# heimrih/polar_code

Measured on AMD Instinct MI355X. Metric: decoded frames/sec, P(128,64)+CRC24 SCL L=8 @ Eb/N0=5 dB; FER match, higher is better.
Workload: dtype f64

## Files before the change

### polar_code_amd/csrc/scl128_lane.hip

```cpp
#ifndef PSCL_LANE_REMAP
#define PSCL_LANE_REMAP 0
#endif
#if PSCL_LANE_REMAP
#define PSCL_LANE_FRAME_MIRROR 0x140
#endif
#include "scl_lane.h"

#ifdef PSCL_LANE_F32_UNIT
using lane_llr_t = float;
#define scl_lane_kernel scl_lane_kernel_f32
#else
using lane_llr_t = double;
#endif

namespace {

#ifndef PSCL_LANE_REG56
#define PSCL_LANE_REG56 1
#endif

#ifndef PSCL_LANE_FRES8
#define PSCL_LANE_FRES8 8
#endif
#ifndef PSCL_LANE_FRES4
#define PSCL_LANE_FRES4 24
#endif

template <int LMAX>
struct LaneLayout {
    static constexpr int G = LMAX;
    static constexpr int F = 64 / G;
    static constexpr int LOG_G = __builtin_ctz(G);
    static constexpr int OFF3 = 0;
    static constexpr int OFF4 = OFF3 + 16 * LMAX;
    static constexpr int OFF5 = OFF4 + 8 * LMAX;
    static constexpr int OFF6 = OFF5 + 4 * LMAX;
    static constexpr int OFFX = PSCL_LANE_REG56 ? OFF4 : OFF6;
    static constexpr int RAW = PSCL_LANE_REG56 ? OFF5 : OFF6 + 2 * LMAX;
    static constexpr int FRES = LMAX == 8 ? PSCL_LANE_FRES8 : PSCL_LANE_FRES4;
    static constexpr int FSTRIDE = RAW + (((FRES - RAW) % 32) + 32) % 32;
    static constexpr int FSTRIDE_FS = FSTRIDE >= 128 ? FSTRIDE : FSTRIDE + 32;
    static constexpr int FSTRIDE_EX = FSTRIDE + 8;
};

__device__ __forceinline__ uint64_t flip_order_key(double q) {
    if (q == 0.0) q = 0.0;
    const uint64_t u = pscl_asu64(q);
    return (u >> 63) ? ~u : (u | 0x8000000000000000ULL);
}

#ifndef PSCL_LANE_CREG4
#define PSCL_LANE_CREG4 1
#endif

#ifndef PSCL_LANE_ABL
#define PSCL_LANE_ABL 0
#endif

#ifndef PSCL_LANE_WAVES_PER_EU
#define PSCL_LANE_WAVES_PER_EU 2
#endif

#ifndef PSCL_LANE_U0T
#define PSCL_LANE_U0T 1
#endif
#ifndef PSCL_LANE_GSPLIT
#define PSCL_LANE_GSPLIT 1
#endif

__device__ __forceinline__ void tx_frame_words(const pscl_decode_params& P, uint64_t fr, uint64_t (&m)[2],
                                               uint64_t (&raw)[2], uint64_t (&x)[2]) {
    const u32x4 rb = philox4x32(u32x4{(uint32_t)fr, (uint32_t)(fr >> 32), 0xffffffffu, 0u}, P.tx_k0, P.tx_k1);
    raw[0] = ((uint64_t)rb.y << 32) | rb.x;
    raw[1] = ((uint64_t)rb.w << 32) | rb.z;
    const int kp = P.tx_kp, nbp = (kp + 7) >> 3, nb = (P.K + 7) >> 3;
    m[0] = kp >= 64 ? raw[0] : (raw[0] & ((1ULL << kp) - 1));
    m[1] = kp > 64 ? (raw[1] & ((kp >= 128) ? ~0ULL : ((1ULL << (kp - 64)) - 1))) : 0;
    uint32_t rem = 0;
    for (int k = 0; k < nbp; ++k) rem ^= P.tx_crctab[k * 256 + (uint32_t)((m[k >> 3] >> (8 * (k & 7))) & 255u)];
    if (P.tx_crc_deg) {
        const uint64_t rw = (uint64_t)rem;
        if (kp < 64) {
            m[0] |= rw << kp;
            if (kp + P.tx_crc_deg > 64) m[1] |= rw >> (64 - kp);
        } else {
            m[1] |= rw << (kp - 64);
        }
    }
    x[0] = x[1] = 0;
    for (int k = 0; k < nb; ++k) {
        const uint32_t v = (uint32_t)((m[k >> 3] >> (8 * (k & 7))) & 255u);
        x[0] ^= P.tx_xtab[(k * 256 + v) * 2];
        x[1] ^= P.tx_xtab[(k * 256 + v) * 2 + 1];
    }
}

#ifndef PSCL_FS_WAVES
#define PSCL_FS_WAVES 3
#endif
#ifndef PSCL_TX_WAVES
#define PSCL_TX_WAVES 3
#endif
template <int LMAX, int CODE, bool FS = false, bool TXF = false, bool FP = false, bool EX = false, bool RL = false>
__global__ void __launch_bounds__(64, TXF ? (LMAX == 8 ? PSCL_TX_WAVES : 2)
                                           : (FS && !FP && !EX && LMAX == 8) ? PSCL_FS_WAVES : PSCL_LANE_WAVES_PER_EU)
scl_lane_kernel(const pscl_decode_params P) {
    static_assert(LMAX == 4 || LMAX == 8, "the lane-per-path decoder is built for L = 4 and 8");
    static_assert(!TXF || (!FS && CODE == 1), "fused TX: plain decodes of the (128,64) code");
    static_assert(!FP || (FS && CODE == 1), "fused post pass: the FS instance of the (128,64) code");
    static_assert(!EX || (!TXF && !FP), "the exact instance: plain re-decodes and forced-bit retry decodes");
    static_assert(!RL || (!FS && !TXF && !FP && !EX), "the row-list form: plain screening decodes");
    using Ly = LaneLayout<LMAX>;
    constexpr int G = Ly::G, F = Ly::F, LOG_G = Ly::LOG_G;
    constexpr int EPL = 16 / G;
    constexpr uint32_t GM = (1u << G) - 1u;
    constexpr int K = kSpecK[CODE], PW = (K + 63) / 64;
    constexpr uint64_t info0 = kSpecInfo[CODE][0], info1 = kSpecInfo[CODE][1];
    extern __shared__ __attribute__((aligned(16))) unsigned char smem[];
    double* const A = reinterpret_cast<double*>(smem);
    const int lane = threadIdx.x & 63;
    constexpr bool REMAP = PSCL_LANE_REMAP && G == 8 && !EX;
    const int rq = (lane >> 2) & 3, inner = (rq == 1 || rq == 2) ? 1 : 0;
    const int fl = REMAP ? 2 * (lane >> 4) + inner : lane >> LOG_G;
    const int p = REMAP ? (lane & 3) + 4 * (rq & 1) : lane & (G - 1);
    const int lane_lo = REMAP ? (lane & ~15) + (inner ? 8 : 0) : lane & ~(G - 1);
    const int lane_hi = REMAP ? (lane & ~15) + (inner ? 4 : 12) : lane_lo + 4;
    auto lane_of = [&](uint32_t q) -> int { return REMAP ? (q < 4u ? lane_lo + (int)q : lane_hi + (int)q - 4) : lane_lo + (int)q; };
    double* const Af = A + fl * (FP ? Ly::FSTRIDE_FS : EX ? Ly::FSTRIDE_EX : Ly::FSTRIDE);
    int* const sl = reinterpret_cast<int*>(Af + Ly::FSTRIDE);
    const uint8_t* const GT = reinterpret_cast<const uint8_t*>(P.epi_table);
    const uint32_t* const ST = reinterpret_cast<const uint32_t*>(GT + 16 * 256);
    auto hiw = [](double m) { return (uint32_t)(pscl_asu64(m) >> 32); };
    constexpr bool BITS = !FS && !EX && PSCL_LANE_BITS;
    constexpr bool PLAIN = !FS && !EX && !TXF;
    constexpr bool U0T = PLAIN && PSCL_LANE_U0T;
    constexpr bool GSPLIT = PLAIN && PSCL_LANE_GSPLIT && (LMAX == 8 || PSCL_LANE_CREG4);
    constexpr double MARGIN = BITS ? PSCL_TAIL2_MARGIN : PSCL_TAIL_ABS_MARGIN;
    auto hiw_up = [&](double m) {
        double r;
        asm("v_fma_f64 %0, %1, %2, %3" : "=v"(r) : "v"(m), "s"(1.0 + 0x1p-40), "v"(MARGIN));
        return hiw(r);
    };
    auto frame_bits = [&](uint64_t m) -> uint32_t {
        if constexpr (REMAP) return ((uint32_t)(m >> lane_lo) & 15u) | (((uint32_t)(m >> lane_hi) & 15u) << 4);
        return (uint32_t)(m >> lane_lo) & GM;
    };

    int cfe = 0, cbe = 0, cpe = 0, cpb = 0;
    int tufe = 0, tube = 0;
    int pdecodes = 0;
    int bpre[PSCL_DL_NSEG + 1];
    int64_t Bn = P.B;
    if constexpr (FS) {
        const int64_t tot = pscl_bucket_prefix(P.bcount, P.bcap, bpre);
        Bn = tot < P.B ? tot : P.B;
    } else if constexpr (EX) {
        if (P.d_count) Bn = *P.d_count < P.B ? (int64_t)*P.d_count : P.B;
    } else if constexpr (RL) {
        Bn = *P.d_count < P.B ? (int64_t)*P.d_count : P.B;
    }
    for (int64_t f0 = (int64_t)blockIdx.x * F; f0 < Bn; f0 += (int64_t)gridDim.x * F) {
        const int64_t fi = f0 + fl;
        const bool fvalid = fi < Bn;
        const int64_t fsafe = fvalid ? fi : f0;
        int64_t f = fi, frow = fsafe;
        int seg0 = 0;
        if constexpr (FS) {
            f = pscl_elist_entry(P, fsafe, bpre);
            seg0 = pscl_bucket_of(f0, bpre);
            frow = P.fidx[f];
        } else if constexpr (EX) {
            if (P.fidx) frow = P.fidx[fsafe];
        } else if constexpr (RL) {
            frow = P.fidx[fsafe];
        }
        constexpr bool RM = CODE == 2;
        const lane_llr_t* chan = reinterpret_cast<const lane_llr_t*>(P.llr) + frow * (RM ? (int64_t)P.rm_E : (int64_t)kN);
        auto chan_at = [&](int i) -> double { return RM ? nr_stage(chan, P.rm_src[i], P.rm_E, kN) : (double)chan[i]; };
        constexpr bool CREG = G == 8 || PSCL_LANE_CREG4 || TXF;
        double c[8 * EPL];
        uint64_t tm[2] = {0, 0}, traw[2] = {0, 0}, tx[2] = {0, 0};
        const uint64_t tfr = TXF ? (uint64_t)(P.tx_frame0 + fsafe) : 0ULL;
        if constexpr (TXF) tx_frame_words(P, tfr, tm, traw, tx);
        auto gen_chan = [&](double* v, uint64_t fr) {
#pragma unroll
            for (int k = 0; k < EPL; ++k)
#pragma unroll
                for (int j = 0; j < 4; ++j) {
                    const uint32_t blk = (uint32_t)(p + G * k + 16 * j);
                    const u32x4 rn = philox4x32(u32x4{(uint32_t)fr, (uint32_t)(fr >> 32), blk, 0u}, P.tx_k0, P.tx_k1);
                    double z[2];
                    bm_pair(((uint64_t)rn.y << 32) | rn.x, ((uint64_t)rn.w << 32) | rn.z, z[0], z[1]);
#pragma unroll
                    for (int h = 0; h < 2; ++h) {
                        const double sym = ((tx[h] >> blk) & 1ULL) ? -1.0 : 1.0;
                        v[8 * k + j + 4 * h] = (sym + P.tx_sigma * z[h]) * P.tx_scale;
                    }
                    __builtin_amdgcn_sched_barrier(0);
                }
        };
        auto load_chan = [&]() {
            if constexpr (TXF) {
                gen_chan(c, tfr);
                if constexpr (BITS)
#pragma unroll
                    for (int m = 0; m < 8 * EPL; ++m) c[m] = c[m] * PSCL_LOG2E_F64;
            } else {
#pragma unroll
                for (int k = 0; k < EPL; ++k)
#pragma unroll
                    for (int m = 0; m < 8; ++m) c[8 * k + m] = BITS ? chan_at(p + G * k + 16 * m) * PSCL_LOG2E_F64
                                                                    : chan_at(p + G * k + 16 * m);
            }
        };
        load_chan();
        uint32_t ah[4 * EPL];
#pragma unroll
        for (int m = 0; m < 4 * EPL; ++m) {
            ah[m] = GSPLIT ? hiw(c[8 * (m >> 2) + (m & 3)]) : 0u;
            if constexpr (GSPLIT) asm volatile("" : "+v"(ah[m]));
        }
        if constexpr (TXF) {
            if (P.tx_upart) {
                uint32_t berr = 0;
                for (int cb = p; 2 * cb < P.tx_kp; cb += G) {
                    const u32x4 rn = philox4x32(u32x4{(uint32_t)tfr, (uint32_t)(tfr >> 32), 0x40000000u + (uint32_t)cb, 0u},
                                                P.tx_k0, P.tx_k1);
                    double z[2];
                    bm_pair(((uint64_t)rn.y << 32) | rn.x, ((uint64_t)rn.w << 32) | rn.z, z[0], z[1]);
#pragma unroll
                    for (int h = 0; h < 2; ++h) {
                        const int q = 2 * cb + h;
                        if (q < P.tx_kp) {
                            const uint32_t bit = (uint32_t)((traw[q >> 6] >> (q & 63)) & 1ULL);
                            const double y = (bit ? -1.0 : 1.0) + P.tx_unc_sigma * z[h];
                            berr += ((y < 0.0) ? 1u : 0u) != bit ? 1u : 0u;
                        }
                    }
                }
                berr = frame_sum<G>(berr);
                if (fvalid && p == 0) {
                    tufe += berr ? 1 : 0;
                    tube += (int)berr;
                }
            }
        }
        double cs = fabs(c[0]);
#pragma unroll
        for (int m = 1; m < 8 * EPL; ++m) cs = cs + fabs(c[m]);
        uint64_t amb = EX ? 0ULL : wmask(!(cs < (BITS ? PSCL_TAIL2_CHAN_SUM : 0x1p25)));
        const uint64_t vmask = wmask(fvalid);

        double metric = 0.0;
        uint64_t u0 = 0, u1 = 0;
        uint32_t tab = 0;
        uint32_t lastbit = 0;
        double r5[4] = {0.0, 0.0, 0.0, 0.0}, r6[2] = {0.0, 0.0};
        uint64_t fm0 = 0, fm1 = 0, fv0 = 0, fv1 = 0;
        int lcnt = 0;
        if constexpr (FS) {
            const uint64_t* fr = P.force + f * 2 * PW;
            fm0 = fr[0];
            fv0 = fr[PW];
            if (PW > 1) {
                fm1 = fr[1];
                fv1 = fr[PW + 1];
            }
            if (seg0 > 0) {
                metric = P.warm_metric[f * PSCL_DL_NSEG + seg0];
                const int lo = 16 * seg0;
                u0 = P.warm_u[2 * f];
                u1 = P.warm_u[2 * f + 1];
                if (lo < 64) {
                    u0 &= (1ULL << lo) - 1ULL;
                    u1 = 0;
                } else {
                    u1 = lo == 64 ? 0ULL : (u1 & ((1ULL << (lo - 64)) - 1ULL));
                }
            }
        }

        auto phase = [&](auto PC) {
            constexpr int phi = decltype(PC)::value;
            constexpr int t = phi & 15;
            constexpr int start = t ? kn - __builtin_ctz((unsigned)t) : ((phi >> 4) ? 3 - __builtin_ctz((unsigned)(phi >> 4)) : 1);
            constexpr bool is_info = ((phi < 64 ? info0 : info1) >> (phi & 63)) & 1;
            constexpr int jb = phi < 64 ? __builtin_popcountll(info0 & ((1ULL << (phi & 63)) - 1))
                                        : __builtin_popcountll(info0) + __builtin_popcountll(info1 & ((1ULL << (phi & 63)) - 1));
            constexpr int cnt = jb >= LOG_G ? LMAX : (1 << jb);
#ifdef PSCL_PHASE_MARKERS
            asm volatile("; PHASE %0" ::"n"(t));
#endif

            if constexpr (start <= 3 && !(PSCL_LANE_ABL & 4)) {
                constexpr bool r1 = phi >= 64, r2 = (phi >> 5) & 1, r3 = (phi >> 4) & 1;
                if constexpr (!CREG && phi > 0) load_chan();
                uint4* const xs = reinterpret_cast<uint4*>(Af + Ly::OFFX);
                if constexpr (r1 || r2 || r3) {
                    uint64_t X1 = 0;
                    uint32_t X2 = 0, X3 = 0;
                    if constexpr (U0T && phi == 64) u0 = polar_transform64(u0);
                    if (r1) X1 = U0T ? u0 : polar_transform64(u0);
                    if (r2) {
                        constexpr int lo = phi - (phi & 31) - 32;
                        X2 = polar_transform32((uint32_t)((lo >= 64 ? u1 : u0) >> (lo & 63)));
                    }
                    if (r3) {
                        constexpr int lo = phi - 16;
                        X3 = polar_transform16((uint32_t)((lo >= 64 ? u1 : u0) >> (lo & 63)) & 0xffffu);
                    }
                    xs[p] = make_uint4((uint32_t)X1, (uint32_t)(X1 >> 32), X2, (X2 >> 16) | (X3 << 16));
                    wave_lds_fence();
                }
                constexpr bool shared2 = !r1 && !r2;
                double d1l[EPL][4], d2s[EPL][2];
#pragma unroll
                for (int h = 0; h < EPL; ++h) {
#pragma unroll
                    for (int m = 0; m < 4; ++m) d1l[h][m] = r1 ? 0.0 : f_minsum(c[8 * h + m], c[8 * h + m + 4]);
#pragma unroll
                    for (int s2 = 0; s2 < 2; ++s2) d2s[h][s2] = shared2 ? f_minsum(d1l[h][s2], d1l[h][s2 + 2]) : 0.0;
                }
                constexpr int npaths = FS ? LMAX : cnt;
#pragma unroll
                for (int q0 = 0; q0 < npaths; ++q0) {
                    const int q = npaths == LMAX ? ((q0 + p) & (LMAX - 1)) : q0;
                    uint64_t x1 = 0, x23 = 0;
                    if constexpr (r1 || r2 || r3) {
                        const uint4 xv = xs[q];
                        x1 = ((uint64_t)xv.y << 32) | xv.x;
                        x23 = ((uint64_t)xv.w << 32) | xv.z;
                    }
                    double d3[EPL];
#pragma unroll
                    for (int h = 0; h < EPL; ++h) {
                        const uint32_t e = (uint32_t)(p + G * h);
                        const uint64_t s1[2] = {r1 ? x1 << (31u - e) : 0ULL, r1 ? x1 << (15u - e) : 0ULL};
                        const uint64_t s2w = r2 ? x23 << (31u - e) : 0ULL;
                        double d1[4];
#pragma unroll
                        for (int m = 0; m < 4; ++m)
                            d1[m] = !r1 ? d1l[h][m]
                                    : GSPLIT ? g_node_bit31_split(c[8 * h + m], ah[4 * h + m], c[8 * h + m + 4],
                                                                  (uint32_t)(s1[m & 1] >> (32 * (m >> 1))))
                                             : g_node_bit31(c[8 * h + m], c[8 * h + m + 4], (uint32_t)(s1[m & 1] >> (32 * (m >> 1))));
                        double d2[2];
#pragma unroll
                        for (int s2 = 0; s2 < 2; ++s2)
                            d2[s2] = shared2 ? d2s[h][s2]
                                             : (r2 ? g_node_bit31(d1[s2], d1[s2 + 2], (uint32_t)(s2w >> (32 * s2))) : f_minsum(d1[s2], d1[s2 + 2]));
                        d3[h] = r3 ? g_node_wbit(d2[0], d2[1], (uint32_t)(x23 >> 32), e + 16) : f_minsum(d2[0], d2[1]);
                    }
#pragma unroll
                    for (int h = 0; h < EPL / 2; ++h)
                        *reinterpret_cast<double2*>(Af + Ly::OFF3 + ((p + G * h) * LMAX + q) * 2) = make_double2(d3[h], d3[h + EPL / 2]);
                }
                wave_lds_fence();
            }
            if constexpr (start <= 6) {
                uint32_t xsb = 0;
                if constexpr (phi && start >= 4) {
                    constexpr int w = 1 << (kn - start), lo = phi - w;
                    static_assert(phi <= 64 || lo >= 64, "u0 is not read bit-wise after phase 64 (PSCL_LANE_U0T)");
                    xsb = polar_transform8((uint32_t)((lo >= 64 ? u1 : u0) >> (lo & 63)) & ((1u << w) - 1u));
                }
                static_for<3>([&](auto DI) {
                    constexpr int D = 4 + decltype(DI)::value;
                    if constexpr (D >= start) {
                        constexpr int W = 1 << (kn - D), HW = W / 2;
                        constexpr int OFF_IN = D == 4 ? Ly::OFF3 : (D == 5 ? Ly::OFF4 : Ly::OFF5);
                        constexpr int OFF_OUT = D == 4 ? Ly::OFF4 : (D == 5 ? Ly::OFF5 : Ly::OFF6);
                        constexpr bool first = D == start || (D == 4 && start < 4);
                        constexpr bool is_g = D == start && phi != 0;
                        if constexpr (PSCL_LANE_REG56 && D == 6) {
#pragma unroll
                            for (int k = 0; k < 2; ++k)
                                r6[k] = is_g ? g_node(r5[k], r5[k + 2], (xsb >> k) & 1u) : f_minsum(r5[k], r5[k + 2]);
                        } else {
                            const int sin = first ? slot_at(tab, D - 1) : p;
                            const int sin_eff = (D == 4 && start <= 3) ? p : sin;
                            const double* in = Af + OFF_IN + sin_eff * 2;
                            double o[W];
#pragma unroll
                            for (int k = 0; k < W; ++k) {
                                const double2 ab = *reinterpret_cast<const double2*>(in + k * LMAX * 2);
                                o[k] = is_g ? g_node(ab.x, ab.y, (xsb >> k) & 1u) : f_minsum(ab.x, ab.y);
                            }
                            if constexpr (PSCL_LANE_REG56 && D == 5) {
#pragma unroll
                                for (int k = 0; k < 4; ++k) r5[k] = o[k];
                            } else {
                                double* out = Af + OFF_OUT + p * 2;
                                if constexpr (HW >= 1) {
#pragma unroll
                                    for (int k = 0; k < (HW ? HW : 1); ++k)
                                        *reinterpret_cast<double2*>(out + k * LMAX * 2) = make_double2(o[k], o[k + HW]);
                                }
                                wave_lds_fence();
                            }
                        }
                    }
                });
                constexpr int s0 = start < 3 ? 3 : start;
                constexpr uint32_t mask = (0xffffu << (4 * (s0 - 3))) & 0xffffu;
                tab = (tab & ~mask) | ((uint32_t)p * 0x1111u & mask);
            }
            const double2 lab = PSCL_LANE_REG56 ? make_double2(r6[0], r6[1])
                                                : *reinterpret_cast<const double2*>(Af + Ly::OFF6 + (start <= 6 ? p : slot_at(tab, 6)) * 2);
            constexpr bool C6 = PSCL_LANE_REG56 && (t % 2 == 0), C5 = PSCL_LANE_REG56 && (t % 4 <= 1);
            auto carry = [&](int src, double (&q5)[4], double (&q6)[2]) {
                if constexpr (C5)
#pragma unroll
                    for (int k = 0; k < 4; ++k) q5[k] = shfl_f64(r5[k], src);
                if constexpr (C6)
#pragma unroll
                    for (int k = 0; k < 2; ++k) q6[k] = shfl_f64(r6[k], src);
            };
            auto take = [&](const double (&q5)[4], const double (&q6)[2]) {
                if constexpr (C5)
#pragma unroll
                    for (int k = 0; k < 4; ++k) r5[k] = q5[k];
                if constexpr (C6)
#pragma unroll
                    for (int k = 0; k < 2; ++k) r6[k] = q6[k];
            };
            const double lam = (phi & 1) ? g_node(lab.x, lab.y, lastbit) : f_minsum(lab.x, lab.y);
            const double Lt = EX ? pscl_softplus_tail_bf(lam, P.exp_table) : BITS ? pscl_softplus_tail2(lam) : pscl_softplus_tail_abs(lam);
            if constexpr (EX) {
                const int ncur = FS ? (1 << lcnt) : cnt;
                const bool live = p < ncur;
                const bool zl = lam == 0.0;
                auto pull_path = [&](int src) {
                    u0 = shfl_u64(u0, src);
                    if constexpr (phi >= 64) u1 = shfl_u64(u1, src);
                    tab = bperm32(tab, src);
                    double q5[4], q6[2];
                    carry(src, q5, q6);
                    take(q5, q6);
                };
                if constexpr (!is_info) {
                    metric = zl ? metric + PSCL_LOGE2 : metric + (relu_neg(lam) + Lt);
                    lastbit = 0;
                    const double pm = shfl_f64(metric, p > 0 ? lane - 1 : lane);
                    if ((wmask(live && pm > metric) & vmask) == 0) return;
                    const double mk = live ? metric : __builtin_inf();
                    uint32_t r = 0;
#pragma unroll
                    for (int sx = 1; sx < G; ++sx) {
                        const double om = shfl_f64(mk, lane ^ sx);
                        r += (om < mk || (om == mk && (p ^ sx) < p)) ? 1u : 0u;
                    }
                    if (live) sl[r] = p;
                    wave_lds_fence();
                    const int src = lane_lo + sl[p & (ncur - 1)];
                    wave_lds_fence();
                    metric = shfl_f64(metric, src);
                    pull_path(src);
                    return;
                }
                const bool neg = lam < 0.0;
                const double mgd = metric + Lt, mbd = metric + (fabs(lam) + Lt);
                double m0 = neg ? mbd : mgd, m1 = neg ? mgd : mbd;
                if (zl) {
                    m0 = metric + PSCL_LOGE2;
                    m1 = m0;
                }
                bool forced = false;
                uint32_t fbit = 0;
                if constexpr (FS) {
                    const uint64_t fmw = jb < 64 ? fm0 : fm1, fvw = jb < 64 ? fv0 : fv1;
                    forced = ((fmw >> (jb & 63)) & 1ULL) != 0;
                    fbit = (uint32_t)((fvw >> (jb & 63)) & 1ULL);
                }
                const double top = shfl_f64(mgd, lane_lo + LMAX - 1), pg = shfl_f64(mgd, p > 0 ? lane - 1 : lane);
                const bool badk = zl || (p > 0 && pg > mgd) || !(mbd > top);
                const bool fast = forced ? ncur == 1 : (ncur == LMAX && frame_bits(wmask(badk)) == 0);
                uint32_t b = forced ? fbit : sign_bit(lam);
                if ((wmask(!fast) & vmask) != 0) {
                    const bool v0 = live && (!forced || fbit == 0u), v1 = live && (!forced || fbit == 1u);
                    const int ncnt = forced ? ncur : (2 * ncur < LMAX ? 2 * ncur : LMAX);
                    const double k0 = v0 ? m0 : __builtin_inf(), k1 = v1 ? m1 : __builtin_inf();
                    uint32_t r0 = k1 < k0 ? 1u : 0u, r1 = k0 <= k1 ? 1u : 0u;
#pragma unroll
                    for (int sx = 1; sx < G; ++sx) {
                        const double o0 = shfl_f64(k0, lane ^ sx), o1 = shfl_f64(k1, lane ^ sx);
                        const bool lt = (p ^ sx) < p;
                        r0 += ((o0 < k0 || (o0 == k0 && lt)) ? 1u : 0u) + ((o1 < k0 || (o1 == k0 && lt)) ? 1u : 0u);
                        r1 += ((o0 < k1 || (o0 == k1 && lt)) ? 1u : 0u) + ((o1 < k1 || (o1 == k1 && lt)) ? 1u : 0u);
                    }
                    if (!fast) {
                        if (v0 && r0 < (uint32_t)ncnt) sl[r0] = 2 * p;
                        if (v1 && r1 < (uint32_t)ncnt) sl[r1] = 2 * p + 1;
                    }
                    wave_lds_fence();
                    const int code = fast ? 2 * p + (int)b : sl[p & (ncnt - 1)];
                    wave_lds_fence();
                    const int src = lane_lo + (code >> 1);
                    b = (uint32_t)code & 1u;
                    const double p0 = shfl_f64(m0, src), p1 = shfl_f64(m1, src);
                    metric = b ? p1 : p0;
                    pull_path(src);
                    if constexpr (FS) lcnt += (!fast && !forced && ncur < LMAX) ? 1 : 0;
                } else {
                    metric = b ? m1 : m0;
                }
                if (phi < 64) u0 |= (uint64_t)b << phi; else u1 |= (uint64_t)b << (phi - 64);
                lastbit = b;
                return;
            }
            if constexpr (!is_info) {
                metric = metric + (relu_neg(lam) + Lt);
                lastbit = 0;
                return;
            }
            const double mg = metric + Lt, mb = mg + fabs(lam);
            const uint32_t gbit = sign_bit(lam);
            if constexpr (FS) {
                const uint64_t fmw = jb < 64 ? fm0 : fm1, fvw = jb < 64 ? fv0 : fv1;
                const bool forced = ((fmw >> (jb & 63)) & 1ULL) != 0;
                const uint32_t fbit = (uint32_t)((fvw >> (jb & 63)) & 1ULL);
                const bool full = !forced && lcnt == LOG_G, grow = !forced && lcnt < LOG_G;
                const int cntf = 1 << lcnt;
                const double m1 = gbit ? mg : mb;
                double nm = forced ? (fbit == gbit ? mg : mb) : (grow ? (gbit ? mb : mg) : mg);
                uint32_t b = forced ? fbit : (grow ? 0u : gbit);
                bool pull = grow && (p & cntf) != 0;
                int src = grow ? lane_of((uint32_t)(p & (cntf - 1))) : lane;
                const uint64_t fullm = wmask(full) & vmask;
                const uint32_t kgu = hiw_up(mg), kb = hiw(mb);
                const uint32_t mx = frame_max<G>(kgu);
                const bool bad = kb <= mx;
                const uint64_t badm = wmask(bad);
                if ((badm & fullm) != 0) {
                    const uint32_t bad8 = frame_bits(badm);
                    if ((wmask(__builtin_popcount(bad8) > 1) & fullm) == 0) {
                        const uint32_t kg = hiw(mg);
                        const uint32_t gmaxh = frame_max<G>(kg);
                        const bool ismax = kg == gmaxh;
                        const uint32_t nmax = frame_sum<G>(ismax ? 1u : 0u);
                        const uint32_t g2u = frame_max<G>(ismax ? 0u : kgu);
                        const uint32_t wu = frame_max<G>(bad ? hiw_up(mb) : 0u);
                        const bool swap = bad8 != 0;
                        amb |= wmask(full && swap && !(nmax == 1u && g2u < gmaxh && wu < gmaxh)) & vmask;
                        if (full && swap && ismax) {
                            pull = true;
                            src = lane_of(__builtin_ctz(bad8 | (1u << G)) & (G - 1));
                        }
                    } else {
                        const uint32_t kg = hiw(mg);
                        bool keep_g, win_b;
                        select_survivors<G, LMAX>(kg, kb, keep_g, win_b);
                        const uint32_t kbu = hiw_up(mb);
                        const uint32_t su = keep_g ? (win_b ? kbu : kgu) : (win_b ? kbu : 0u);
                        const uint32_t nmk = keep_g ? (win_b ? 0xffffffffu : kb) : kg;
                        const uint32_t nsurv = frame_sum<G>((keep_g ? 1u : 0u) + (win_b ? 1u : 0u));
                        const uint32_t smax = frame_max<G>(su), nmin = frame_min<G>(nmk);
                        amb |= wmask(full && !(nsurv == (uint32_t)LMAX && nmin > smax)) & vmask;
                        const uint32_t f8 = frame_bits(wmask(!keep_g)), w8 = frame_bits(wmask(win_b));
                        const uint32_t jj = __builtin_popcount(f8 & ((1u << p) - 1u));
                        const int rsrc = lane_of(nth_set_bit8(w8, jj));
                        if (full && !keep_g) {
                            pull = true;
                            src = rsrc;
                        }
                    }
                }
                if (wmask(pull) != 0) {
                    const uint64_t pubm = pscl_asu64(full ? mb : m1);
                    const uint32_t tw = tab | ((full ? (gbit ^ 1u) : 1u) << 31);
                    const uint64_t pm = shfl_u64(pubm, src);
                    const uint64_t pu0 = shfl_u64(u0, src);
                    const uint64_t pu1 = phi >= 64 ? shfl_u64(u1, src) : 0ULL;
                    const uint32_t ptw = bperm32(tw, src);
                    double q5[4], q6[2];
                    carry(src, q5, q6);
                    if (pull) {
                        nm = pscl_asf64(pm);
                        u0 = pu0;
                        u1 = pu1;
                        tab = ptw & 0x7fffffffu;
                        b = ptw >> 31;
                        take(q5, q6);
                    }
                }
                metric = nm;
                if (phi < 64) u0 |= (uint64_t)b << phi; else u1 |= (uint64_t)b << (phi - 64);
                lastbit = b;
                lcnt += grow ? 1 : 0;
                return;
            }
            if constexpr (cnt < LMAX) {
                const double m0 = gbit ? mb : mg, m1 = gbit ? mg : mb;
                const int src = lane_of((uint32_t)(p & (cnt - 1)));
                const uint32_t b = (p & cnt) ? 1u : 0u;
                const uint64_t pm1 = shfl_u64(pscl_asu64(m1), src);
                metric = b ? pscl_asf64(pm1) : m0;
                u0 = shfl_u64(u0, src);
                if (phi >= 64) u1 = shfl_u64(u1, src);
                tab = bperm32(tab, src);
                double q5[4], q6[2];
                carry(src, q5, q6);
                take(q5, q6);
                if (phi < 64) u0 |= (uint64_t)b << phi; else u1 |= (uint64_t)b << (phi - 64);
                lastbit = b;
                return;
            }
            const uint32_t kgu = hiw_up(mg), kb = hiw(mb);
            const uint32_t mx = frame_max<G>(kgu);
            const bool bad = kb <= mx;
            const uint64_t badm = wmask(bad);
#ifdef PSCL_STATS
            const bool one = (wmask(__builtin_popcount(frame_bits(badm)) > 1) & vmask) == 0;
            if (lane == 0 && P.counters) {
                atomicAdd(reinterpret_cast<unsigned long long*>(P.counters) + ((badm & vmask) == 0 ? 12 : (one ? 13 : 14)), 1ULL);
            }
#endif
            metric = mg;
            uint32_t b = gbit;
            if (!(PSCL_LANE_ABL & 2) && ((badm & vmask) != 0 || (PSCL_LANE_ABL & 1))) {
                const uint32_t bad8 = frame_bits(badm);
                bool pull;
                int src;
#if PSCL_LANE_SWAP
                if (!(PSCL_LANE_ABL & 1) && (wmask(__builtin_popcount(bad8) > 1) & vmask) == 0) {
                    const uint32_t kg = hiw(mg);
                    const uint32_t gmaxh = frame_max<G>(kg);
                    const bool ismax = kg == gmaxh;
                    const uint32_t nmax = __builtin_popcount(frame_bits(wmask(ismax)));
                    const bool g2ok = ismax || kgu < gmaxh;
                    const bool wok = !bad || hiw_up(mb) < gmaxh;
                    const bool swap = bad8 != 0;
                    amb |= wmask(swap && !(nmax == 1u && g2ok && wok)) & vmask;
                    src = lane_of(__builtin_ctz(bad8 | (1u << G)) & (G - 1));
                    pull = swap && ismax;
                } else
#endif
                {
                    const uint32_t kg = hiw(mg);
                    uint32_t rg, rbb;
                    rank_children<G>(kg, kb, rg, rbb);
                    const bool keep_g = rg < (uint32_t)LMAX;
                    const uint32_t f8 = frame_bits(wmask(!keep_g));
                    const uint32_t d = __builtin_popcount(f8);
                    const bool win_b = rbb < d;
                    const uint32_t w8 = frame_bits(wmask(win_b));
#if defined(PSCL_STATS) && PSCL_STATS == 2
                    {
                        const uint32_t dw = frame_sum<G>(win_b ? 1u : 0u);
                        const uint32_t nb = __builtin_popcount(bad8);
                        unsigned long long* C = reinterpret_cast<unsigned long long*>(P.counters);
                        if (p == 0 && fvalid && C) {
                            atomicAdd(C + 16 + (dw > 8u ? 8u : dw), 1ULL);
                            atomicAdd(C + 25 + nb, 1ULL);
                        }
                        uint32_t md = 0;
                        for (uint32_t k = 1; k <= 8; ++k)
                            if (wmask(dw >= k) & vmask) md = k;
                        if (lane == 0 && C) atomicAdd(C + 34 + md, 1ULL);
                    }
#endif
                    const uint32_t kbu = hiw_up(mb);
                    const uint32_t su = keep_g ? (win_b ? kbu : kgu) : (win_b ? kbu : 0u);
                    const uint32_t nm = keep_g ? (win_b ? 0xffffffffu : kb) : kg;
                    const uint32_t smax = frame_max<G>(su);
                    amb |= wmask(!((uint32_t)__builtin_popcount(w8) == d && nm > smax)) & vmask;
                    src = lane_of(matched_winner<G>(f8, w8, win_b, (uint32_t)p));
                    pull = !keep_g;
                }
                const int srce = pull ? src : lane;
                const uint64_t pmb = shfl_u64(pscl_asu64(mb), srce);
                const uint32_t ptw = bperm32(tab | ((gbit ^ 1u) << 31), srce);
                u0 = shfl_u64(u0, srce);
                if constexpr (phi >= 64) u1 = shfl_u64(u1, srce);
                tab = ptw & 0x7fffffffu;
                double q5[4], q6[2];
                carry(srce, q5, q6);
                take(q5, q6);
                if (pull) {
                    metric = pscl_asf64(pmb);
                    b = ptw >> 31;
                }
            }
            if (phi < 64) u0 |= (uint64_t)b << phi; else u1 |= (uint64_t)b << (phi - 64);
            lastbit = b;
        };
        if constexpr (FS) {
            auto seg = [&](auto SB) {
                static_for<16>([&](auto TC) { phase(std::integral_constant<int, decltype(SB)::value * 16 + decltype(TC)::value>{}); });
            };
            using std::integral_constant;
            switch (seg0) {
                case 0: seg(integral_constant<int, 0>{}); [[fallthrough]];
                case 1: seg(integral_constant<int, 1>{}); [[fallthrough]];
                case 2: seg(integral_constant<int, 2>{}); [[fallthrough]];
                case 3: seg(integral_constant<int, 3>{}); [[fallthrough]];
                case 4: seg(integral_constant<int, 4>{}); [[fallthrough]];
                case 5: seg(integral_constant<int, 5>{}); [[fallthrough]];
                case 6: seg(integral_constant<int, 6>{}); [[fallthrough]];
                default: seg(integral_constant<int, 7>{});
            }
        } else {
            static_for<kN>([&](auto PC) { phase(PC); });
        }

        auto fused_post = [&](bool x_amb, bool x_live, uint32_t x_keyb, uint32_t x_kbest, uint64_t x_ib0, uint64_t x_ib1,
                              uint64_t x_u0, uint64_t x_u1, int64_t x_frow, int64_t e, bool x_valid) {
            static_assert(!REMAP, "the fused post pass assumes frames of G consecutive lanes");
            const pscl_post_params& Q = P.fp;
            constexpr int NC = K / G;
            const uint32_t fl = (x_kbest < (uint32_t)LMAX ? PSCL_FLAG_CRC_PASS : 0u) | (x_kbest & (uint32_t)(LMAX - 1));
            const bool mine = x_valid && !x_amb;
            int nt = 0;
            uint64_t t0 = 0, t1 = 0;
            if (mine) {
                nt = Q.ntried[e];
                t0 = Q.tried[2 * e];
                t1 = Q.tried[2 * e + 1];
            }
            const uint32_t bfb = frame_bits(wmask(x_live && x_keyb == x_kbest));
            const int bsrc = lane_lo + (bfb ? __builtin_ctz(bfb) : 0);
            const uint64_t bi0 = shfl_u64(x_ib0, bsrc), bi1 = PW > 1 ? shfl_u64(x_ib1, bsrc) : 0ULL;
            const uint64_t bu0 = shfl_u64(x_u0, bsrc), bu1 = shfl_u64(x_u1, bsrc);
            if (mine && p == 0) {
                Q.best[x_frow * PW] = bi0;
                if (PW > 1) Q.best[x_frow * PW + 1] = bi1;
                Q.flags[x_frow] = (uint8_t)fl;
                if (Q.attempts) Q.attempts[x_frow] = nt + 1;
                ++pdecodes;
            }
            const bool more = mine && !(fl & PSCL_FLAG_CRC_PASS) && nt < Q.rounds;
            if (wmask(more) == 0) return;
            wave_lds_fence();
            {
                const double* crow = P.llr + x_frow * kN;
#pragma unroll
                for (int j = 0; j < kN / G; ++j) Af[p + G * j] = crow[p + G * j];
            }
            wave_lds_fence();
            auto stage = [](uint64_t x, int st) {
                const uint64_t M = st == 1 ? 0x5555555555555555ULL : st == 2 ? 0x3333333333333333ULL
                                 : st == 4 ? 0x0f0f0f0f0f0f0f0fULL : st == 8 ? 0x00ff00ff00ff00ffULL
                                 : st == 16 ? 0x0000ffff0000ffffULL : 0x00000000ffffffffULL;
                return x ^ ((x >> st) & M);
            };
            uint64_t X0 = bu0, X1 = bu1;
#pragma unroll
            for (int mm = 1; mm < kn; ++mm) {
                X0 = stage(X0, 1 << (mm - 1));
                X1 = stage(X1, 1 << (mm - 1));
            }
            static_for<kn>([&](auto DC) {
                constexpr int lw2 = kn - 1 - decltype(DC)::value, w2 = 1 << lw2;
                const bool act_l = w2 >= G || (p & w2) == 0;
                if (act_l) {
#pragma unroll 2
                    for (int j = 0; j < kN / G; ++j) {
                        const int q = p + G * j;
                        if (w2 >= G && (q & w2)) continue;
                        const double a = Af[q], b = Af[q + w2];
                        const uint32_t bit = (uint32_t)(((q >> 6) ? X1 : X0) >> (q & 63)) & 1u;
                        Af[q] = f_minsum(a, b);
                        Af[q + w2] = g_node(a, b, bit);
                    }
                }
                wave_lds_fence();
                if constexpr (lw2 > 0) {
                    X0 = stage(X0, w2 >> 1);
                    X1 = stage(X1, w2 >> 1);
                }
            });
            float qv[NC];
            double as = 0.0;
            uint64_t bk = ~0ULL;
            int bj = 0x7fffffff;
            auto seen_j = [&](int j) { return (((j < 64 ? t0 : t1) >> (j & 63)) & 1ULL) != 0; };
            auto argmin = [&]() {
                bk = ~0ULL;
                bj = 0x7fffffff;
#pragma unroll
                for (int i = 0; i < NC; ++i) {
                    const int j = p + G * i;
                    const uint64_t key = seen_j(j) ? ~0ULL : flip_order_key((double)qv[i]);
                    if (key < bk) {
                        bk = key;
                        bj = j;
                    }
                }
#pragma unroll
                for (int sft = 1; sft < G; sft <<= 1) {
                    const uint64_t ok = shfl_u64(bk, lane ^ sft);
                    const int oj = __shfl(bj, lane ^ sft);
                    if (ok < bk || (ok == bk && oj < bj)) {
                        bk = ok;
                        bj = oj;
                    }
                }
            };
            auto argmin_exact = [&]() {
                bk = ~0ULL;
                bj = 0x7fffffff;
#pragma unroll 1
                for (int i = 0; i < NC; ++i) {
                    const int j = p + G * i;
                    double qx = 0.0;
#pragma unroll 1
                    for (int k = 0; k < K; ++k) qx = qx + fabs(Af[Q.info_set[k]]) * Q.beta[k * K + j];
                    const uint64_t key = seen_j(j) ? ~0ULL : flip_order_key(qx);
                    if (key < bk) {
                        bk = key;
                        bj = j;
                    }
                }
#pragma unroll
                for (int sft = 1; sft < G; sft <<= 1) {
                    const uint64_t ok = shfl_u64(bk, lane ^ sft);
                    const int oj = __shfl(bj, lane ^ sft);
                    if (ok < bk || (ok == bk && oj < bj)) {
                        bk = ok;
// ... 380 lines not shown
```

### polar_code_amd/csrc/scl_lane.h

```cpp
#ifndef PSCL_SCL_LANE_H
#define PSCL_SCL_LANE_H

#include "scl128_impl.h"

#ifndef PSCL_LANE_SWAP
#define PSCL_LANE_SWAP 1
#endif


#ifndef PSCL_LANE_BITS
#define PSCL_LANE_BITS 1
#endif

namespace {

constexpr int kQX1 = 0xB1, kQX2 = 0x4E, kQX3 = 0x1B, kQID = 0xE4, kHMIR = 0x141;
#ifndef PSCL_LANE_FRAME_MIRROR
#define PSCL_LANE_FRAME_MIRROR 0x141
#endif
constexpr int kFMIR = PSCL_LANE_FRAME_MIRROR;

template <int CTRL>
__device__ __forceinline__ uint32_t dpp32(uint32_t v) {
    return (uint32_t)__builtin_amdgcn_mov_dpp((int)v, CTRL, 0xF, 0xF, true);
}

template <int CTRL>
__device__ __forceinline__ void rank_pair(uint32_t og, uint32_t ob, uint32_t kg, uint32_t kb, uint32_t& rg, uint32_t& rb) {
    uint32_t t;
    asm volatile(
        "s_nop 1\n\t"
        "v_sub_co_u32_dpp %0, vcc, %3, %5 quad_perm:[%7,%8,%9,%10] row_mask:0xf bank_mask:0xf\n\t"
        "v_addc_co_u32 %1, vcc, 0, %1, vcc\n\t"
        "v_sub_co_u32_dpp %0, vcc, %4, %5 quad_perm:[%7,%8,%9,%10] row_mask:0xf bank_mask:0xf\n\t"
        "v_addc_co_u32 %1, vcc, 0, %1, vcc\n\t"
        "v_sub_co_u32_dpp %0, vcc, %3, %6 quad_perm:[%7,%8,%9,%10] row_mask:0xf bank_mask:0xf\n\t"
        "v_addc_co_u32 %2, vcc, 0, %2, vcc\n\t"
        "v_sub_co_u32_dpp %0, vcc, %4, %6 quad_perm:[%7,%8,%9,%10] row_mask:0xf bank_mask:0xf\n\t"
        "v_addc_co_u32 %2, vcc, 0, %2, vcc"
        : "=&v"(t), "+v"(rg), "+v"(rb)
        : "v"(og), "v"(ob), "v"(kg), "v"(kb), "i"(CTRL & 3), "i"((CTRL >> 2) & 3), "i"((CTRL >> 4) & 3),
          "i"((CTRL >> 6) & 3)
        : "vcc");
}

template <int CTRL>
__device__ __forceinline__ void rank3(uint32_t og, uint32_t ob, uint32_t kg, uint32_t kb, uint32_t& rg, uint32_t& rbb) {
    uint32_t t;
    asm volatile(
        "s_nop 1\n\t"
        "v_sub_co_u32_dpp %0, vcc, %3, %5 quad_perm:[%7,%8,%9,%10] row_mask:0xf bank_mask:0xf\n\t"
        "v_addc_co_u32 %1, vcc, 0, %1, vcc\n\t"
        "v_sub_co_u32_dpp %0, vcc, %4, %5 quad_perm:[%7,%8,%9,%10] row_mask:0xf bank_mask:0xf\n\t"
        "v_addc_co_u32 %1, vcc, 0, %1, vcc\n\t"
        "v_sub_co_u32_dpp %0, vcc, %4, %6 quad_perm:[%7,%8,%9,%10] row_mask:0xf bank_mask:0xf\n\t"
        "v_addc_co_u32 %2, vcc, 0, %2, vcc"
        : "=&v"(t), "+v"(rg), "+v"(rbb)
        : "v"(og), "v"(ob), "v"(kg), "v"(kb), "i"(CTRL & 3), "i"((CTRL >> 2) & 3), "i"((CTRL >> 4) & 3),
          "i"((CTRL >> 6) & 3)
        : "vcc");
}

constexpr int kRMIR = 0x140;

__device__ __forceinline__ uint32_t xrow32(uint32_t v) { return (uint32_t)__shfl_xor((int)v, 16); }

template <int G>
__device__ __forceinline__ uint32_t frame_max(uint32_t v) {
    uint32_t o = dpp32<kQX1>(v);
    v = o > v ? o : v;
    o = dpp32<kQX2>(v);
    v = o > v ? o : v;
    if constexpr (G >= 8) {
        o = dpp32<G >= 16 ? kHMIR : kFMIR>(v);
        v = o > v ? o : v;
    }
    if constexpr (G >= 16) {
        o = dpp32<kRMIR>(v);
        v = o > v ? o : v;
    }
    if constexpr (G == 32) {
        o = xrow32(v);
        v = o > v ? o : v;
    }
    return v;
}
template <int G>
__device__ __forceinline__ uint32_t frame_min(uint32_t v) {
    uint32_t o = dpp32<kQX1>(v);
    v = o < v ? o : v;
    o = dpp32<kQX2>(v);
    v = o < v ? o : v;
    if constexpr (G >= 8) {
        o = dpp32<G >= 16 ? kHMIR : kFMIR>(v);
        v = o < v ? o : v;
    }
    if constexpr (G >= 16) {
        o = dpp32<kRMIR>(v);
        v = o < v ? o : v;
    }
    if constexpr (G == 32) {
        o = xrow32(v);
        v = o < v ? o : v;
    }
    return v;
}
template <int G>
__device__ __forceinline__ uint32_t frame_sum(uint32_t v) {
    v += dpp32<kQX1>(v);
    v += dpp32<kQX2>(v);
    if constexpr (G >= 8) v += dpp32<G >= 16 ? kHMIR : kFMIR>(v);
    if constexpr (G >= 16) v += dpp32<kRMIR>(v);
    if constexpr (G == 32) v += xrow32(v);
    return v;
}
template <int G>
__device__ __forceinline__ uint32_t frame_or(uint32_t v) {
    v |= dpp32<kQX1>(v);
    v |= dpp32<kQX2>(v);
    if constexpr (G >= 8) v |= dpp32<G >= 16 ? kHMIR : kFMIR>(v);
    if constexpr (G >= 16) v |= dpp32<kRMIR>(v);
    if constexpr (G == 32) v |= xrow32(v);
    return v;
}

#ifndef PSCL_LANE_RANK3
#define PSCL_LANE_RANK3 1
#endif
template <int G, int LMAX>
__device__ __forceinline__ void select_survivors(uint32_t kg, uint32_t kb, bool& keep_g, bool& win_b) {
#if PSCL_LANE_RANK3
    uint32_t rg = 0, rbb = 0;
    rank3<kQX1>(kg, kb, kg, kb, rg, rbb);
    rank3<kQX2>(kg, kb, kg, kb, rg, rbb);
    rank3<kQX3>(kg, kb, kg, kb, rg, rbb);
    if constexpr (G >= 8) {
        const uint32_t mkg = dpp32<G >= 16 ? kHMIR : kFMIR>(kg), mkb = dpp32<G >= 16 ? kHMIR : kFMIR>(kb);
        rank3<kQID>(mkg, mkb, kg, kb, rg, rbb);
        rank3<kQX1>(mkg, mkb, kg, kb, rg, rbb);
        rank3<kQX2>(mkg, mkb, kg, kb, rg, rbb);
        rank3<kQX3>(mkg, mkb, kg, kb, rg, rbb);
    }
    auto quads16 = [&](uint32_t ok, uint32_t ob) {
        rank3<kQID>(ok, ob, kg, kb, rg, rbb);
        rank3<kQX1>(ok, ob, kg, kb, rg, rbb);
        rank3<kQX2>(ok, ob, kg, kb, rg, rbb);
        rank3<kQX3>(ok, ob, kg, kb, rg, rbb);
    };
    if constexpr (G >= 16) {
        quads16(dpp32<kRMIR>(kg), dpp32<kRMIR>(kb));
        quads16(dpp32<kRMIR>(dpp32<kHMIR>(kg)), dpp32<kRMIR>(dpp32<kHMIR>(kb)));
    }
    if constexpr (G == 32) {
        const uint32_t xg = xrow32(kg), xb = xrow32(kb);
        quads16(xg, xb);
        quads16(dpp32<kHMIR>(xg), dpp32<kHMIR>(xb));
        quads16(dpp32<kRMIR>(xg), dpp32<kRMIR>(xb));
        quads16(dpp32<kRMIR>(dpp32<kHMIR>(xg)), dpp32<kRMIR>(dpp32<kHMIR>(xb)));
    }
    keep_g = rg < (uint32_t)LMAX;
    const uint32_t d = frame_sum<G>(keep_g ? 0u : 1u);
    win_b = rbb < d;
#else
    static_assert(G <= 8, "the two-rank selection is built for frames of at most 8 lanes");
    uint32_t rg = 0, rb = kg < kb ? 1u : 0u;
    rank_pair<kQX1>(kg, kb, kg, kb, rg, rb);
    rank_pair<kQX2>(kg, kb, kg, kb, rg, rb);
    rank_pair<kQX3>(kg, kb, kg, kb, rg, rb);
    if constexpr (G == 8) {
        const uint32_t mkg = dpp32<kFMIR>(kg), mkb = dpp32<kFMIR>(kb);
        rank_pair<kQID>(mkg, mkb, kg, kb, rg, rb);
        rank_pair<kQX1>(mkg, mkb, kg, kb, rg, rb);
        rank_pair<kQX2>(mkg, mkb, kg, kb, rg, rb);
        rank_pair<kQX3>(mkg, mkb, kg, kb, rg, rb);
    }
    keep_g = rg < (uint32_t)LMAX;
    win_b = rb < (uint32_t)LMAX;
#endif
}

#define PSCL_RANK3_BLK(OG, OB, QP)                                                                  \
    "v_sub_co_u32_dpp %[t], vcc, " OG ", %[kg] quad_perm:" QP " row_mask:0xf bank_mask:0xf\n\t"          \
    "v_addc_co_u32 %[rg], vcc, 0, %[rg], vcc\n\t"                                                         \
    "v_sub_co_u32_dpp %[t], vcc, " OB ", %[kg] quad_perm:" QP " row_mask:0xf bank_mask:0xf\n\t"          \
    "v_addc_co_u32 %[rg], vcc, 0, %[rg], vcc\n\t"                                                         \
    "v_sub_co_u32_dpp %[t], vcc, " OB ", %[kb] quad_perm:" QP " row_mask:0xf bank_mask:0xf\n\t"          \
    "v_addc_co_u32 %[rbb], vcc, 0, %[rbb], vcc\n\t"
#if PSCL_LANE_FRAME_MIRROR == 0x140
#define PSCL_FRAME_MIRROR_DPP "row_mirror"
#else
#define PSCL_FRAME_MIRROR_DPP "row_half_mirror"
#endif
template <int G>
__device__ __forceinline__ void rank_children(uint32_t kg, uint32_t kb, uint32_t& rg, uint32_t& rbb) {
    static_assert(G == 4 || G == 8, "the fused rank counts are built for frames of 4 or 8 lanes");
    uint32_t t;
    rg = 0;
    rbb = 0;
    if constexpr (G == 4) {
        asm volatile("s_nop 1\n\t"
                     PSCL_RANK3_BLK("%[kg]", "%[kb]", "[1,0,3,2]")
                     PSCL_RANK3_BLK("%[kg]", "%[kb]", "[2,3,0,1]")
                     PSCL_RANK3_BLK("%[kg]", "%[kb]", "[3,2,1,0]")
                     : [t] "=&v"(t), [rg] "+v"(rg), [rbb] "+v"(rbb)
                     : [kg] "v"(kg), [kb] "v"(kb)
                     : "vcc");
    } else {
        uint32_t mkg, mkb;
        asm volatile("s_nop 1\n\t"
                     "v_mov_b32_dpp %[mkg], %[kg] " PSCL_FRAME_MIRROR_DPP " row_mask:0xf bank_mask:0xf\n\t"
                     "v_mov_b32_dpp %[mkb], %[kb] " PSCL_FRAME_MIRROR_DPP " row_mask:0xf bank_mask:0xf\n\t"
                     PSCL_RANK3_BLK("%[kg]", "%[kb]", "[1,0,3,2]")
                     PSCL_RANK3_BLK("%[kg]", "%[kb]", "[2,3,0,1]")
                     PSCL_RANK3_BLK("%[kg]", "%[kb]", "[3,2,1,0]")
                     PSCL_RANK3_BLK("%[mkg]", "%[mkb]", "[0,1,2,3]")
                     PSCL_RANK3_BLK("%[mkg]", "%[mkb]", "[1,0,3,2]")
                     PSCL_RANK3_BLK("%[mkg]", "%[mkb]", "[2,3,0,1]")
                     PSCL_RANK3_BLK("%[mkg]", "%[mkb]", "[3,2,1,0]")
                     : [t] "=&v"(t), [rg] "+v"(rg), [rbb] "+v"(rbb), [mkg] "=&v"(mkg), [mkb] "=&v"(mkb)
                     : [kg] "v"(kg), [kb] "v"(kb)
                     : "vcc");
    }
}
#undef PSCL_RANK3_BLK

__device__ __forceinline__ uint32_t nth_set_bit16(uint32_t m, uint32_t j);
__device__ __forceinline__ uint32_t nth_set_bit32(uint32_t m, uint32_t j) {
    const uint32_t c16 = __builtin_popcount(m & 0xffffu);
    const bool h16 = j >= c16;
    return (h16 ? 16u : 0u) + nth_set_bit16(h16 ? (m >> 16) : (m & 0xffffu), h16 ? j - c16 : j);
}

__device__ __forceinline__ uint32_t nth_set_bit16(uint32_t m, uint32_t j) {
    const uint32_t c8 = __builtin_popcount(m & 255u);
    const bool h8 = j >= c8;
    j = h8 ? j - c8 : j;
    m = h8 ? (m >> 8) : (m & 255u);
    const uint32_t c4 = __builtin_popcount(m & 15u);
    const bool h4 = j >= c4;
    j = h4 ? j - c4 : j;
    m = h4 ? (m >> 4) : (m & 15u);
    const uint32_t c2 = __builtin_popcount(m & 3u);
    const bool h2 = j >= c2;
    j = h2 ? j - c2 : j;
    m = h2 ? (m >> 2) : m;
    const bool h1 = j >= (m & 1u);
    return (h8 ? 8u : 0u) + (h4 ? 4u : 0u) + (h2 ? 2u : 0u) + (h1 ? 1u : 0u);
}

__device__ __forceinline__ uint32_t nth_set_bit8(uint32_t m, uint32_t j) {
    const uint32_t c4 = __builtin_popcount(m & 15u);
    const bool h4 = j >= c4;
    j = h4 ? j - c4 : j;
    m = h4 ? (m >> 4) : (m & 15u);
    const uint32_t c2 = __builtin_popcount(m & 3u);
    const bool h2 = j >= c2;
    j = h2 ? j - c2 : j;
    m = h2 ? (m >> 2) : m;
    const bool h1 = j >= (m & 1u);
    return (h4 ? 4u : 0u) + (h2 ? 2u : 0u) + (h1 ? 1u : 0u);
}

template <int G>
__device__ __forceinline__ uint32_t matched_winner(uint32_t f8, uint32_t w8, bool win, uint32_t p) {
    static_assert(G == 4 || G == 8, "the packed matching holds one nibble per lane of a frame of 4 or 8");
    const uint32_t below = (1u << p) - 1u;
    const uint32_t j = __builtin_popcount(f8 & below);
    const uint32_t r = __builtin_popcount(w8 & below);
    const uint32_t W = frame_or<G>(win ? p << (4u * r) : 0u);
    return (W >> (4u * j)) & (uint32_t)(G - 1);
}

}

#endif
```

Baseline: 609.0 million.

## Plan partial sums at compile time from frozen-bit windows for g-nodes

At compile time, the information-bit window for each phase is used to build a plan that computes each g-node's partial-sum sign as an XOR of shifted decision bits, skipping the runtime polar transform. Nodes whose partial-sum set is empty become a plain addition. A cost model keeps the transform wherever the plan would be more expensive. Separately, the ambiguity-mask computation is rewritten as bitwise combinations of wave masks instead of a single boolean mask. This removes ALU work on the per-phase critical path but adds template complexity and static asserts tied to the specific code sets.

```diff
diff --git a/polar_code_amd/csrc/scl128_lane.hip b/polar_code_amd/csrc/scl128_lane.hip
--- a/polar_code_amd/csrc/scl128_lane.hip
+++ b/polar_code_amd/csrc/scl128_lane.hip
@@ -67,6 +67,43 @@
 #ifndef PSCL_LANE_GSPLIT
 #define PSCL_LANE_GSPLIT 1
 #endif
+
+template <uint32_t IW, int W, int LO>
+__device__ __forceinline__ void psplan_row_masks(uint32_t uw, uint32_t (&psm)[8]) {
+    uint32_t mb[8] = {0, 0, 0, 0, 0, 0, 0, 0};
+    static_for<W>([&](auto IC) {
+        constexpr int i = decltype(IC)::value;
+        if constexpr ((IW >> i) & 1u) mb[i] = uw << (31 - ((LO + i) & 31));
+    });
+    static_for<W>([&](auto KC) {
+        constexpr int k = decltype(KC)::value;
+        constexpr uint32_t S = psplan_set(IW, W, k);
+        psm[k] = 0;
+        if constexpr (S != 0) psm[k] = psplan_mask<S>(mb);
+    });
+}
+template <uint32_t IW, int W, int K>
+__device__ __forceinline__ double psplan_g_node(double a, double b, const uint32_t (&psm)[8]) {
+    if constexpr (psplan_set(IW, W, K) == 0) return b + a;
+    else return g_node_bit31(a, b, psm[K]);
+}
+template <uint32_t IW, int LO>
+__device__ __forceinline__ void psplan_row_reg(uint32_t uw, const double (&r5)[4], double (&r6)[2]) {
+    uint32_t psm[8];
+    psplan_row_masks<IW, 2, LO>(uw, psm);
+    r6[0] = psplan_g_node<IW, 2, 0>(r5[0], r5[2], psm);
+    r6[1] = psplan_g_node<IW, 2, 1>(r5[1], r5[3], psm);
+}
+template <uint32_t IW, int W, int LO, int LMAX>
+__device__ __forceinline__ void psplan_row_lds(uint32_t uw, const double* in, double (&o)[W]) {
+    uint32_t psm[8];
+    psplan_row_masks<IW, W, LO>(uw, psm);
+    static_for<W>([&](auto KC) {
+        constexpr int k = decltype(KC)::value;
+        const double2 ab = *reinterpret_cast<const double2*>(in + k * LMAX * 2);
+        o[k] = psplan_g_node<IW, W, k>(ab.x, ab.y, psm);
+    });
+}
 
 __device__ __forceinline__ void tx_frame_words(const pscl_decode_params& P, uint64_t fr, uint64_t (&m)[2],
                                                uint64_t (&raw)[2], uint64_t (&x)[2]) {
@@ -134,6 +171,7 @@
     constexpr bool BITS = !FS && !EX && PSCL_LANE_BITS;
     constexpr bool PLAIN = !FS && !EX && !TXF;
     constexpr bool U0T = PLAIN && PSCL_LANE_U0T;
+    constexpr bool PSPLAN = PLAIN && PSCL_LANE_PSPLAN;
     constexpr bool GSPLIT = PLAIN && PSCL_LANE_GSPLIT && (LMAX == 8 || PSCL_LANE_CREG4);
     constexpr double MARGIN = BITS ? PSCL_TAIL2_MARGIN : PSCL_TAIL_ABS_MARGIN;
     auto hiw_up = [&](double m) {
@@ -359,10 +397,18 @@
             }
             if constexpr (start <= 6) {
                 uint32_t xsb = 0;
+                constexpr bool GW = phi && start >= 4 && start <= 6;
+                constexpr uint32_t iw = GW ? psplan_window(info0, info1, phi) : 0u;
+                constexpr bool PSP = GW && PSPLAN && psplan_planned(iw, GW ? psplan_width(phi) : 2);
                 if constexpr (phi && start >= 4) {
                     constexpr int w = 1 << (kn - start), lo = phi - w;
                     static_assert(phi <= 64 || lo >= 64, "u0 is not read bit-wise after phase 64 (PSCL_LANE_U0T)");
-                    xsb = polar_transform8((uint32_t)((lo >= 64 ? u1 : u0) >> (lo & 63)) & ((1u << w) - 1u));
+                    if constexpr (!PSP) {
+                        xsb = polar_transform8((uint32_t)((lo >= 64 ? u1 : u0) >> (lo & 63)) & ((1u << w) - 1u));
+                    } else {
+                        static_assert(w == psplan_width(phi) && psplan_proved(iw, w), "the partial-sum plan");
+                        xsb = (uint32_t)((lo >= 64 ? u1 : u0) >> (32 * ((lo & 63) >> 5)));
+                    }
                 }
                 static_for<3>([&](auto DI) {
                     constexpr int D = 4 + decltype(DI)::value;
@@ -373,18 +419,26 @@
                         constexpr bool first = D == start || (D == 4 && start < 4);
                         constexpr bool is_g = D == start && phi != 0;
                         if constexpr (PSCL_LANE_REG56 && D == 6) {
-#pragma unroll
-                            for (int k = 0; k < 2; ++k)
-                                r6[k] = is_g ? g_node(r5[k], r5[k + 2], (xsb >> k) & 1u) : f_minsum(r5[k], r5[k + 2]);
+                            if constexpr (!(PSP && is_g)) {
+#pragma unroll
+                                for (int k = 0; k < 2; ++k)
+                                    r6[k] = is_g ? g_node(r5[k], r5[k + 2], (xsb >> k) & 1u) : f_minsum(r5[k], r5[k + 2]);
+                            } else {
+                                psplan_row_reg<iw, phi - 2>(xsb, r5, r6);
+                            }
                         } else {
                             const int sin = first ? slot_at(tab, D - 1) : p;
                             const int sin_eff = (D == 4 && start <= 3) ? p : sin;
                             const double* in = Af + OFF_IN + sin_eff * 2;
                             double o[W];
-#pragma unroll
-                            for (int k = 0; k < W; ++k) {
-                                const double2 ab = *reinterpret_cast<const double2*>(in + k * LMAX * 2);
-                                o[k] = is_g ? g_node(ab.x, ab.y, (xsb >> k) & 1u) : f_minsum(ab.x, ab.y);
+                            if constexpr (!(PSP && is_g)) {
+#pragma unroll
+                                for (int k = 0; k < W; ++k) {
+                                    const double2 ab = *reinterpret_cast<const double2*>(in + k * LMAX * 2);
+                                    o[k] = is_g ? g_node(ab.x, ab.y, (xsb >> k) & 1u) : f_minsum(ab.x, ab.y);
+                                }
+                            } else {
+                                psplan_row_lds<iw, W, phi - W, LMAX>(xsb, in, o);
                             }
                             if constexpr (PSCL_LANE_REG56 && D == 5) {
 #pragma unroll
@@ -630,7 +684,13 @@
                     const bool g2ok = ismax || kgu < gmaxh;
                     const bool wok = !bad || hiw_up(mb) < gmaxh;
                     const bool swap = bad8 != 0;
-                    amb |= wmask(swap && !(nmax == 1u && g2ok && wok)) & vmask;
+                    if constexpr (!PSPLAN) {
+                        amb |= wmask(swap && !(nmax == 1u && g2ok && wok)) & vmask;
+                    } else {
+                        const uint64_t g2okm = wmask(ismax) | wmask(kgu < gmaxh);
+                        const uint64_t wokm = ~badm | wmask(hiw_up(mb) < gmaxh);
+                        amb |= wmask(swap) & ~(wmask(nmax == 1u) & g2okm & wokm) & vmask;
+                    }
                     src = lane_of(__builtin_ctz(bad8 | (1u << G)) & (G - 1));
                     pull = swap && ismax;
                 } else
@@ -663,7 +723,10 @@
                     const uint32_t su = keep_g ? (win_b ? kbu : kgu) : (win_b ? kbu : 0u);
                     const uint32_t nm = keep_g ? (win_b ? 0xffffffffu : kb) : kg;
                     const uint32_t smax = frame_max<G>(su);
-                    amb |= wmask(!((uint32_t)__builtin_popcount(w8) == d && nm > smax)) & vmask;
+                    if constexpr (!PSPLAN)
+                        amb |= wmask(!((uint32_t)__builtin_popcount(w8) == d && nm > smax)) & vmask;
+                    else
+                        amb |= ~(wmask((uint32_t)__builtin_popcount(w8) == d) & wmask(nm > smax)) & vmask;
                     src = lane_of(matched_winner<G>(f8, w8, win_b, (uint32_t)p));
                     pull = !keep_g;
                 }
diff --git a/polar_code_amd/csrc/scl_lane.h b/polar_code_amd/csrc/scl_lane.h
--- a/polar_code_amd/csrc/scl_lane.h
+++ b/polar_code_amd/csrc/scl_lane.h
@@ -12,7 +12,83 @@
 #define PSCL_LANE_BITS 1
 #endif
 
+#ifndef PSCL_LANE_PSPLAN
+#define PSCL_LANE_PSPLAN 1
+#endif
+
 namespace {
+
+constexpr int psplan_width(int phi) { return (phi & 15) & -(phi & 15); }
+constexpr uint32_t psplan_window(uint64_t info0, uint64_t info1, int phi) {
+    const int w = psplan_width(phi), lo = phi - w;
+    return (uint32_t)((lo >= 64 ? info1 : info0) >> (lo & 63)) & ((1u << w) - 1u);
+}
+constexpr uint32_t psplan_set(uint32_t iw, int w, int k) {
+    uint32_t s = 0;
+    for (int i = 0; i < w; ++i)
+        if (((iw >> i) & 1u) && (i & k) == k) s |= 1u << i;
+    return s;
+}
+constexpr uint32_t psplan_transform8(uint32_t x) {
+    x ^= (x >> 1) & 0x55u;
+    x ^= (x >> 2) & 0x33u;
+    x ^= (x >> 4) & 0x0fu;
+    return x;
+}
+constexpr bool psplan_proved(uint32_t iw, int w) {
+    for (uint32_t v = 0; v < (1u << w); ++v) {
+        if (v & ~iw) continue;
+        const uint32_t x = psplan_transform8(v);
+        for (int k = 0; k < w; ++k) {
+            uint32_t par = 0;
+            for (uint32_t m = v & psplan_set(iw, w, k); m; m &= m - 1u) par ^= 1u;
+            if (par != ((x >> k) & 1u)) return false;
+        }
+    }
+    return true;
+}
+constexpr int psplan_cost_transform(int w) { return 2 + 2 * (w == 8 ? 3 : w == 4 ? 2 : 1) + 2 * w; }
+constexpr int psplan_cost(uint32_t iw, int w) {
+    uint32_t seen[64] = {};
+    int nseen = 0, cost = 0;
+    for (uint32_t m = iw; m; m &= m - 1u) ++cost;
+    for (int k = 0; k < w; ++k) {
+        uint32_t s = psplan_set(iw, w, k);
+        if (s) ++cost;
+        for (; s & (s - 1u); s &= s - 1u) {
+            bool dup = false;
+            for (int j = 0; j < nseen; ++j) dup = dup || seen[j] == s;
+            if (!dup) {
+                seen[nseen++] = s;
+                ++cost;
+            }
+        }
+    }
+    return cost;
+}
+constexpr bool psplan_planned(uint32_t iw, int w) { return psplan_cost(iw, w) < psplan_cost_transform(w); }
+constexpr int psplan_total(uint64_t info0, uint64_t info1) {
+    int tot = 0;
+    for (int phi = 2; phi < 128; phi += 2) {
+        if ((phi & 15) == 0) continue;
+        const int w = psplan_width(phi);
+        const uint32_t iw = psplan_window(info0, info1, phi);
+        tot += psplan_planned(iw, w) ? psplan_cost(iw, w) : psplan_cost_transform(w);
+    }
+    return tot;
+}
+constexpr int psplan_kept(uint64_t info0, uint64_t info1) {
+    int n = 0;
+    for (int phi = 2; phi < 128; phi += 2)
+        if ((phi & 15) != 0 && !psplan_planned(psplan_window(info0, info1, phi), psplan_width(phi))) ++n;
+    return n;
+}
+static_assert(psplan_total(0, 0) == 0 && psplan_kept(0, 0) == 0, "no information bit: every node is b + a");
+static_assert(psplan_total(kSpecInfo[1][0], kSpecInfo[1][1]) == 270 && psplan_kept(kSpecInfo[1][0], kSpecInfo[1][1]) == 0,
+              "partial-sum plan of the (128,64) set");
+static_assert(psplan_total(kSpecInfo[2][0], kSpecInfo[2][1]) == 378 && psplan_kept(kSpecInfo[2][0], kSpecInfo[2][1]) == 1 &&
+                  !psplan_planned(psplan_window(kSpecInfo[2][0], kSpecInfo[2][1], 120), 8),
+              "partial-sum plan of the (128,88) set: phase 120 keeps the transform");
 
 constexpr int kQX1 = 0xB1, kQX2 = 0x4E, kQX3 = 0x1B, kQID = 0xE4, kHMIR = 0x141;
 #ifndef PSCL_LANE_FRAME_MIRROR
@@ -271,6 +347,15 @@
     return (W >> (4u * j)) & (uint32_t)(G - 1);
 }
 
-}
-
-#endif
+template <uint32_t S>
+__device__ __forceinline__ uint32_t psplan_mask(const uint32_t (&mb)[8]) {
+    static_assert(S != 0 && S < 256u, "a non-empty set of window positions");
+    if constexpr ((S & (S - 1u)) == 0)
+        return mb[__builtin_ctz(S)];
+    else
+        return psplan_mask<(S & (S - 1u))>(mb) ^ mb[__builtin_ctz(S)];
+}
+
+}
+
+#endif
```

Result: faster. 623.4 million (median of 6 runs) (+2.4%).
